# evanwang1990/FMwR

Measured on AMD Instinct MI355X. Metric: training examples/sec, 10Mx1M sparse FM SGD, higher is better.
Workload: dtype f32

## Files before the change

### fmwr_amd/_lib.py

```python
import ctypes as C
import os

_PKG = os.path.dirname(os.path.abspath(__file__))
LIB_PATH = os.environ.get("FMX_LIB_PATH") or os.path.join(_PKG, "libfmx.so")

OK, ERR_INVALID, ERR_HIP, ERR_NOGPU, ERR_STATE = 0, 1, 2, 3, 4
TASK_CLASSIFICATION, TASK_REGRESSION, TASK_RANKING = 10, 20, 30
SOLVER_MCMC, SOLVER_ALS, SOLVER_SGD, SOLVER_FTRL, SOLVER_TDAP = 100, 200, 300, 500, 600
MODE_SEQUENTIAL, MODE_MINIBATCH = 0, 1
LINK_NONE, LINK_LOGISTIC, LINK_CLAMP, LINK_PROBIT = 0, 1, 2, 3
DIV_REL_SCORE, DIV_REL_MINMAX = 0, 1
SIM_COSINE, SIM_DOT = 0, 1
REDUCE_MEAN, REDUCE_SUM = 0, 1
COLUMNS_UNIFORM, COLUMNS_ZIPF = 1, 2
EVAL_LL, EVAL_AUC, EVAL_ACC, EVAL_RMSE, EVAL_MSE, EVAL_MAE = 0, 111, 222, 333, 444, 555
EVAL_PAIR_ACC, EVAL_BPR = 666, 777
KERNEL_ROWS_FORWARD, KERNEL_COLS_UPDATE, KERNEL_SCALAR, KERNEL_SEQ, KERNEL_ALS_SWEEP = 0, 1, 2, 3, 4

SYMBOLS = [
    "fmx_last_error", "fmx_device_count", "fmx_config_default", "fmx_engine_create", "fmx_engine_destroy", "fmx_set_params",
    "fmx_get_params", "fmx_engine_save", "fmx_engine_load", "fmx_matrix_from_rlist", "fmx_matrix_from_dgc", "fmx_matrix_from_csr", "fmx_matrix_synthetic", "fmx_matrix_synthetic_fields", "fmx_matrix_synthetic_iid", "fmx_matrix_synthetic_ragged", "fmx_matrix_synthetic_values", "fmx_train_stream", "fmx_matrix_set_labels", "fmx_matrix_set_fields", "fmx_matrix_destroy",
    "fmx_matrix_info", "fmx_matrix_export", "fmx_matrix_scales", "fmx_matrix_normalize", "fmx_predict", "fmx_train", "fmx_train_grid", "fmx_train_order", "fmx_num_batches",
    "fmx_step", "fmx_grad", "fmx_grad_buffer", "fmx_grad_elem_bytes", "fmx_grad_layout", "fmx_grad_begin", "fmx_grad_chunk", "fmx_apply_chunk", "fmx_apply", "fmx_sync", "fmx_stream", "fmx_predict_device",
    "fmx_als_plan_info", "fmx_als_tiled_info", "fmx_als_order_info", "fmx_als_carry_q", "fmx_als_vsweep", "fmx_mcmc_vsweep", "fmx_als_train", "fmx_mcmc_train", "fmx_mcmc_train_from", "fmx_mcmc_v_hyper", "fmx_evaluate", "fmx_train_tracked", "fmx_trace_size", "fmx_trace_get", "fmx_trace_params",
# ... 32 lines not shown
SPLIT_NO_PART = 0xFFFFFFFF
MET_VALUES, MET_COUNTS = 6, 4
MET_AUC, MET_LOGLOSS, MET_ACCURACY, MET_BRIER, MET_MEAN_PRED, MET_MEAN_LABEL = 0, 1, 2, 3, 4, 5
MET_MSE, MET_RMSE, MET_MAE, MET_MEAN_ERR = 0, 1, 2, 3
MET_ROWS, MET_POSITIVES, MET_PAIRS2, MET_CORRECT = 0, 1, 2, 3
CAL_NONE, CAL_PLATT, CAL_STEPS = 0, 1, 2
BINS_WIDTH, BINS_MASS = 0, 1
CAL_VALUES = 4
CAL_ECE, CAL_MCE, CAL_BRIER, CAL_LOGLOSS = 0, 1, 2, 3


TEST_HOOKS = ["fmx_debug_fail_next_plan_build", "fmx_debug_fail_next_comm_init", "fmx_debug_lose_next_seq_multiplier", "fmx_debug_stall_next_persistent_sweep",
              "fmx_debug_contrib_summary_chunk", "fmx_debug_foldin_slab", "fmx_debug_heldout_limits", "fmx_debug_pairs_hard_chunk", "fmx_debug_lists_limits", "fmx_debug_diversify_limits", "fmx_debug_neighbors_limits", "fmx_debug_interactions_limits", "fmx_debug_metrics_limits", "fmx_debug_take_limits", "fmx_debug_calibrate_limits", "fmx_debug_columns_limits", "fmx_debug_join_limits", "fmx_debug_bins_limits", "fmx_debug_matrix_flags", "fmx_debug_cols_launches",
              "fmx_debug_long_launches", "fmx_debug_rows_launches", "fmx_debug_rows_merged_launches",
              "fmx_debug_rows_sched_launches", "fmx_debug_rows_sched_id_limit", "fmx_debug_rows_sched_export",
              "fmx_debug_rows_pace_launches", "fmx_debug_rows_pace_trace",
              "fmx_debug_rows_clock_launches", "fmx_debug_rows_clock_records_of", "fmx_debug_rows_clock_poison"]


class Config(C.Structure):
    _fields_ = [
        ("struct_size", C.c_uint32), ("task", C.c_int32), ("solver", C.c_int32), ("num_factor", C.c_int32),
        ("keep_w0", C.c_int32), ("keep_w1", C.c_int32),
        ("l2_w0", C.c_double), ("l1_w1", C.c_double), ("l2_w1", C.c_double), ("l1_v", C.c_double), ("l2_v", C.c_double),
        ("learn_rate", C.c_double),
        ("alpha_w", C.c_double), ("alpha_v", C.c_double), ("beta_w", C.c_double), ("beta_v", C.c_double),
        ("random_step", C.c_int32), ("mode", C.c_int32), ("batch_rows", C.c_int64),
        ("min_target", C.c_double), ("max_target", C.c_double),
        ("device", C.c_int32), ("batch_reduce", C.c_int32), ("gamma", C.c_double), ("tile_rows", C.c_int64),
        ("state_fp64", C.c_int32), ("exchange_chunks", C.c_int32), ("n_gpus", C.c_int32), ("als_max_levels", C.c_int32), ("seq_reassociate", C.c_int32), ("gpus_share_device", C.c_int32),
    ]
# ... 128 lines not shown
```

### fmwr_amd/csrc/fm_batch_kernels.hip

```cpp
#include <atomic>
#include <mutex>
#include <utility>
#include <vector>

#include "fmx_internal.h"
#include "fm_probit.h"
#include "fmx_test_hooks.h"

#ifndef FMX_U
#define FMX_U 4
#endif
#ifndef FMX_SPARSE_WAVES
#define FMX_SPARSE_WAVES 4
#endif
#ifndef FMX_DENSE_WAVES
#define FMX_DENSE_WAVES 4
#endif
#ifndef FMX_U_LARGE
#define FMX_U_LARGE 4
#endif
#ifndef FMX_U_SMALL
#define FMX_U_SMALL 8
#endif

// ... 453 lines not shown
  }
  if constexpr (TRAIN) {
    __syncthreads();
    if (tid % 64 == 0) {
      const int s = tid / 64;
      if (R0 + (int64_t)s * NG < a.nrows) {
        double g0 = 0.0, q0 = 0.0;
        for (int i = 0; i < NG; ++i) { const double m = red[s * NG + i]; g0 += m; q0 += m * m; }
        a.partials[2 * ((size_t)blockIdx.x * MERGE_SLOTS + s)] = g0;
        a.partials[2 * ((size_t)blockIdx.x * MERGE_SLOTS + s) + 1] = q0;
      }
    }
  }
}

constexpr int64_t PACE_STEP_CYCLES = 2120;

__device__ __forceinline__ void pace_sleep(int units) {
  switch (units) {
    case 3: __builtin_amdgcn_s_sleep(3); break;
    case 4: __builtin_amdgcn_s_sleep(4); break;
    case 5: __builtin_amdgcn_s_sleep(5); break;
    case 6: __builtin_amdgcn_s_sleep(6); break;
    case 8: __builtin_amdgcn_s_sleep(8); break;
    case 9: __builtin_amdgcn_s_sleep(9); break;
    case 10: __builtin_amdgcn_s_sleep(10); break;
    case 12: __builtin_amdgcn_s_sleep(12); break;
    case 15: __builtin_amdgcn_s_sleep(15); break;
    case 16: __builtin_amdgcn_s_sleep(16); break;
    case 24: __builtin_amdgcn_s_sleep(24); break;
    case 20: __builtin_amdgcn_s_sleep(20); break;
// ... 11 lines not shown
#define FMX_ROWS_PACE_CLOCK_EVERY 24
#endif
#ifndef FMX_ROWS_PACE_CLOCK_LEAD
#define FMX_ROWS_PACE_CLOCK_LEAD 0.5
#endif
#ifndef FMX_ROWS_PACE_CLOCK_SLEEP
#define FMX_ROWS_PACE_CLOCK_SLEEP 30
#endif
#ifndef FMX_ROWS_PACE_CLOCK_GAIN
#define FMX_ROWS_PACE_CLOCK_GAIN 1.00
#endif
static_assert((int64_t)((SCHED_STAGE_STEPS - 1) / FMX_ROWS_PACE_CLOCK_EVERY) * 3 * FMX_ROWS_PACE_CLOCK_SLEEP * 64 * 10 <= SCHED_STAGE_STEPS * PACE_STEP_CYCLES, "clock checks x the longest sleep: at most a tenth of the longest block's walk");
static_assert((int64_t)((120 - 1) / FMX_ROWS_PACE_CLOCK_EVERY) * 3 * FMX_ROWS_PACE_CLOCK_SLEEP * 64 * 10 <= 120 * PACE_STEP_CYCLES, "the same for the headline's 120-step blocks");
static_assert(FMX_ROWS_PACE_CLOCK_GAIN > 0.0 && FMX_ROWS_PACE_CLOCK_GAIN <= 1.0, "a gain above 1 would hold a launch to a pace slower than the one observed");

template <bool DEAL, bool PACED, bool TRACE>
__global__ __launch_bounds__(WG_THREADS, 4) void fm_rows_sched_k(RowsArgs a, Hyper h) {
  using T = float;
  constexpr int LPR = 4, VEC = 4, KP = LPR * VEC;
  constexpr int NG = WG_THREADS / LPR;
  constexpr int PER = MERGE_STAGE / WG_THREADS;
  static_assert(MERGE_STAGE == SCHED_STAGE_STEPS * NG && MERGE_SLOTS == 4, "the stage holds SCHED_STAGE_STEPS steps of one word per lane group");
  __shared__ uint32_t stage[MERGE_STAGE];
  __shared__ double red[MERGE_RPW];
  __shared__ uint32_t places[DEAL ? NG : 1];

  const int tid = threadIdx.x;
  const int gid = tid / LPR;
  const int lig = tid % LPR;
  const int64_t R0 = (int64_t)blockIdx.x * MERGE_RPW;
  const uint32_t w_hi = a.sched_dir[blockIdx.x + 1];
  uint32_t w_lo = a.sched_dir[blockIdx.x];
  if constexpr (DEAL) {
    const bool hdr = w_hi - w_lo >= (uint32_t)NG;
    if (tid < NG) places[tid] = hdr ? a.sched[(size_t)w_lo + tid] : 0u;
    w_lo += hdr ? (uint32_t)NG : 0u;
  }
  const int cnt = (w_hi - w_lo < (uint32_t)MERGE_STAGE) ? (int)(w_hi - w_lo) : MERGE_STAGE;
  const int steps = cnt / NG;
  {
    uint32_t id[PER];
// ... 37 lines not shown
      const uint64_t planted = __hip_atomic_load(rec + 1, __ATOMIC_RELAXED, __HIP_MEMORY_SCOPE_AGENT);
      const uint64_t ticks = sums & ((1ull << CLK_TICK_BITS) - 1), done = sums >> CLK_TICK_BITS;
      if (planted) target = (uint32_t)planted;
      else if (done) {
        const double q8 = (double)a.clk_gain_q10 * 0.25 * (double)ticks / (double)done;
        target = q8 < 4294967295.0 ? (uint32_t)q8 : 0xFFFFFFFFu;
      }
    }
    clk_target = (int64_t)(uint32_t)__builtin_amdgcn_readfirstlane((int)target);
    if (clk_target) clk_at = a.pace_every;
    if (blockIdx.x == 0 && tid < 8 && a.clk_zero)
      __hip_atomic_store(a.clk + (size_t)(((a.clk_write + 1) % 3) * 8 + tid) * CLK_LINE, (uint64_t)0, __ATOMIC_RELAXED, __HIP_MEMORY_SCOPE_AGENT);
    clk_t0 = __builtin_amdgcn_s_memrealtime();
  }
  uint64_t* trace = nullptr;
  if constexpr (TRACE) trace = a.pace_trace + ((size_t)blockIdx.x * (WG_THREADS / 64) + tid / 64) * PACE_TRACE_WORDS;
  for (int t = 0; t < steps; ++t) {
    if constexpr (TRACE) {
      if ((t & 15) == 0 && (tid & 63) == 0) trace[1 + (t >> 4)] = __builtin_amdgcn_s_memrealtime();
    }
    const uint32_t wd = mine[t * NG];
    const bool live = wd != SCHED_BUBBLE;
    const uint32_t c = wd & SCHED_MAX_P;
    const int esl = live ? (int)(wd >> 30) : MERGE_SLOTS;
    const float4 vv = buf_row(v_rsrc, live ? (c << vsh) + lane_off : BUF_SKIP, T());
    const T wv = buf_elem(w_rsrc, live ? c << wsh : BUF_SKIP, T());
    const double x = 1.0;
    const double wx = (double)wv * x;
    double tmp[VEC], tsq[VEC];
    slice_get(vv, tmp);
#pragma unroll
    for (int i = 0; i < VEC; ++i) { tmp[i] = tmp[i] * x; tsq[i] = tmp[i] * tmp[i]; }
#pragma unroll
    for (int s = 0; s < MERGE_SLOTS; ++s) {
      if (esl == s) {
        if (k1) lin[s] += wx;
#pragma unroll
        for (int i = 0; i < VEC; ++i) { sm[s][i] += tmp[i]; qm[s][i] += tsq[i]; }
      }
    }
    if constexpr (PACED) {
      if (t == clk_at) {
        clk_at += a.pace_every;
        const int64_t gone = (int64_t)((__builtin_amdgcn_s_memrealtime() - clk_t0) << 10);
        const int64_t done = 4 * (t + 1), lead = a.pace_lead;
        const int level = (done - 3 * lead) * clk_target > gone ? 3 : (done - 2 * lead) * clk_target > gone ? 2 : (done - lead) * clk_target > gone ? 1 : 0;
        if (level) { pace_sleep(level * a.pace_sleep); pace_slept += 1 + (level << 16); }
      }
    }
  }
  if constexpr (PACED) {
    if (tid == 0) {
      const uint64_t ticks = __builtin_amdgcn_s_memrealtime() - clk_t0;
      (void)__hip_atomic_fetch_add(a.clk + (size_t)(a.clk_write * 8 + (int)(blockIdx.x & 7u)) * CLK_LINE,
                                   (ticks & ((1ull << CLK_TICK_BITS) - 1)) | (uint64_t)steps << CLK_TICK_BITS, __ATOMIC_RELAXED, __HIP_MEMORY_SCOPE_AGENT);
    }
  }
  if constexpr (TRACE) {
    if ((tid & 63) == 0) {
      trace[1 + ((steps + 15) >> 4)] = __builtin_amdgcn_s_memrealtime();
      trace[0] = (uint64_t)(__builtin_amdgcn_s_getreg((31 << 11) | 20) & 15u) | (uint64_t)steps << 8 | (uint64_t)pace_slept << 32;
    }
// ... 22 lines not shown
      *reinterpret_cast<float4*>(reinterpret_cast<T*>(a.S) + (size_t)row * KP + lig * VEC) = srow;
      if (lig == 0) reinterpret_cast<T*>(a.amul)[row] = (T)mult;
    }
    if (lig == 0) red[at] = mult;
  }
  __syncthreads();
  if (tid % 64 == 0) {
    const int s = tid / 64;
    if (R0 + (int64_t)s * NG < a.nrows) {
      double g0 = 0.0, q0 = 0.0;
      for (int i = 0; i < NG; ++i) { const double m = red[s * NG + i]; g0 += m; q0 += m * m; }
      a.partials[2 * ((size_t)blockIdx.x * MERGE_SLOTS + s)] = g0;
      a.partials[2 * ((size_t)blockIdx.x * MERGE_SLOTS + s) + 1] = q0;
    }
  }
}

template <typename T, int LPR, bool TRAIN>
__global__ __launch_bounds__(WG_THREADS) void fm_rows_forward_dyn_k(RowsArgs a, Hyper h) {
  using vec_t = typename Slice<T>::vec;
  constexpr int VEC = Slice<T>::N;
  constexpr int KP = LPR * VEC;
  constexpr int GROUPS = WG_THREADS / LPR;
  constexpr int RPW = 4 * GROUPS;
  constexpr int RU = FMX_U_LARGE;
  constexpr int PER = (RU + LPR - 1) / LPR;
  __shared__ int next_row;
  __shared__ double red[TRAIN ? RPW : 1];
  const int tid = threadIdx.x;
  const int grp = tid / LPR, lig = tid % LPR;
  const int lane0 = (tid & 63) - lig;
// ... 463 lines not shown
void rows_sched_count_build() { g_rows_sched[2]++; }
static int rows_sched_mode() {
  static const int v = [] { const char* s = getenv("FMX_ROWS_SCHED"); return s ? atoi(s) : (getenv("FMX_ROWS_MERGE") ? 0 : FMX_ROWS_SCHED_DEFAULT); }();
  return v;
}
static int rows_sched_policy() {
  static const int v = [] {
    const char* s = getenv("FMX_ROWS_SCHED_POLICY");
    if (!s) return (int)FMX_ROWS_SCHED_POLICY_DEFAULT;
    return s[0] == 'm' ? (int)SCHED_MERGE : s[0] == 'd' ? (int)SCHED_DEAL : (int)FMX_ROWS_SCHED_POLICY_DEFAULT;
  }();
  return v;
}

#ifndef FMX_ROWS_PACE_DEFAULT
#define FMX_ROWS_PACE_DEFAULT 3
#endif
static std::atomic<int64_t> g_rows_pace[2];
void debug_rows_pace_launches(int64_t out[2]) {
  for (int i = 0; i < 2; ++i) out[i] = g_rows_pace[i].load();
}
static std::atomic<int64_t> g_rows_clock[2];
void debug_rows_clock_launches(int64_t out[2]) {
  for (int i = 0; i < 2; ++i) out[i] = g_rows_clock[i].load();
}
static int rows_pace_mode() {
  static const int v = [] { const char* s = getenv("FMX_ROWS_PACE"); const int m = s ? atoi(s) : FMX_ROWS_PACE_DEFAULT; return (m == 0 || m == 3 || m == 4) ? m : FMX_ROWS_PACE_DEFAULT; }();
  return v;
}
static bool rows_pace_trace_on() { static const bool v = [] { const char* s = getenv("FMX_ROWS_PACE_TRACE"); return s && s[0] == '1'; }(); return v; }
struct ClockTune { int every, lead_q2, sleep, gain_q10; };
static const ClockTune& rows_clock_tune() {
  static const ClockTune v = [] {
    ClockTune t{FMX_ROWS_PACE_CLOCK_EVERY, (int)(FMX_ROWS_PACE_CLOCK_LEAD * 4.0 + 0.5), FMX_ROWS_PACE_CLOCK_SLEEP, (int)(FMX_ROWS_PACE_CLOCK_GAIN * 1024.0 + 0.5)};
    int ev = 0, sl = 0;
    double ld = -1.0, g = 0.0;
    const char* s = getenv("FMX_ROWS_PACE_CLOCK_TUNE");
    if (s && sscanf(s, "%d,%lf,%d,%lf", &ev, &ld, &sl, &g) == 4 && ev >= 2 && ev <= 64 && ld >= 0.0 && ld <= 64.0 && (sl == 3 || sl == 4 || sl == 5 || sl == 8 || sl == 10 || sl == 20 || sl == 30 || sl == 40) && g > 0.0 && g <= 1.0)
      t = ClockTune{ev, (int)(ld * 4.0 + 0.5), sl, (int)(g * 1024.0 + 0.5)};
    return t;
  }();
  return v;
// ... 28 lines not shown
}

static int launch_rows_sched(fmx_engine* e, const RowsArgs& a_in, bool* ran) {
  *ran = false;
  if (a_in.sched_state == 0) return FMX_OK;
  int policy = 0;
  if (!rows_sched_wanted(e, a_in, &policy)) return FMX_OK;
  if (a_in.sched_state != 1 || !a_in.sched || !a_in.sched_dir) { g_rows_sched[1]++; return FMX_OK; }
  RowsArgs a = a_in;
  a.sched_vbytes = (uint32_t)((uint64_t)e->p * (uint64_t)a.vs * sizeof(float));
  a.sched_wbytes = (uint32_t)((((uint64_t)e->p - 1) * (uint64_t)a.ws + 1) * sizeof(float));
  const int64_t grid = (a.nrows + MERGE_RPW - 1) / MERGE_RPW;
  FMX_CHECK(grid < (1LL << 31), FMX_ERR_INVALID, "rows_forward: grid too large (%lld)", (long long)grid);
  const bool traced = rows_pace_trace_on();
  using SchedKernel = void (*)(RowsArgs, Hyper);
  static const SchedKernel instance[2][2][2] = {
      {{fm_rows_sched_k<false, false, false>, fm_rows_sched_k<false, false, true>}, {fm_rows_sched_k<false, true, false>, fm_rows_sched_k<false, true, true>}},
      {{fm_rows_sched_k<true, false, false>, fm_rows_sched_k<true, false, true>}, {fm_rows_sched_k<true, true, false>, fm_rows_sched_k<true, true, true>}}};
  const int deal = a.sched_deal ? 1 : 0;
  bool paced = false;
  if (rows_pace_mode() != 0 && e->rows_clock != nullptr) {
    constexpr int MAX_DEV = 64;
    static std::atomic<int64_t> resident_dev[MAX_DEV][2][2];
    std::atomic<int64_t>& resident = resident_dev[(e->cfg.device >= 0 && e->cfg.device < MAX_DEV) ? e->cfg.device : 0][deal][traced ? 1 : 0];
    int64_t r = resident.load();
    if (r == 0) {
      hipDeviceProp_t pr{};
      int per = 0;
      if (hipGetDeviceProperties(&pr, e->cfg.device) == hipSuccess && pr.multiProcessorCount > 0 &&
          hipOccupancyMaxActiveBlocksPerMultiprocessor(&per, instance[deal][1][traced ? 1 : 0], WG_THREADS, 0) == hipSuccess && per > 0)
        r = (int64_t)per * pr.multiProcessorCount;
      else r = -1;
      resident.store(r);
    }
    paced = r > 0 && grid <= r;
  }
  bool with_target = false;
  if (paced) {
    const ClockTune& ct = rows_clock_tune();
    const int64_t n = e->rows_clock_launches;
    with_target = e->rows_clock_poisoned || (e->rows_clock_prev && e->rows_clock_uid == a.mat_uid && e->rows_clock_gen == a.mat_gen && e->rows_clock_nrows == a.nrows);
    a.clk = e->rows_clock;
    a.clk_write = (int)(n % 3);
    a.clk_read = with_target ? (int)((n + 2) % 3) : -1;
    a.clk_zero = e->rows_clock_poisoned ? 0 : 1;
// ... 6 lines not shown
      FMX_HIP(hipStreamSynchronize(e->stream));
    }
  }
  if (traced) {
    const int64_t waves = grid * (WG_THREADS / 64);
    if (waves > e->rows_pace_trace_cap) {
      FMX_HIP(hipStreamSynchronize(e->stream));
      (void)hipFree(e->rows_pace_trace); e->rows_pace_trace = nullptr; e->rows_pace_trace_cap = 0;
      FMX_HIP(hipMalloc(&e->rows_pace_trace, (size_t)waves * PACE_TRACE_WORDS * sizeof(uint64_t)));
      e->rows_pace_trace_cap = waves;
    }
    FMX_HIP(hipMemsetAsync(e->rows_pace_trace, 0, (size_t)waves * PACE_TRACE_WORDS * sizeof(uint64_t), e->stream));
    e->rows_pace_trace_waves = waves;
    a.pace_trace = e->rows_pace_trace;
  }
  hipLaunchKernelGGL(instance[deal][paced ? 1 : 0][traced ? 1 : 0], dim3((unsigned)grid), dim3(WG_THREADS), 0, e->stream, a, e->hyper);
  FMX_HIP(hipGetLastError());
  if (paced) {
    ++e->rows_clock_launches;
    e->rows_clock_prev = 1; e->rows_clock_uid = a.mat_uid; e->rows_clock_gen = a.mat_gen; e->rows_clock_nrows = a.nrows;
    g_rows_clock[with_target ? 0 : 1]++;
  }
  g_rows_pace[paced ? 0 : 1]++;
  g_rows_sched[0]++;
  *ran = true;
  return FMX_OK;
}

int launch_rows_forward(fmx_engine* e, const RowsArgs& a_in, bool train, bool fp64_tables) {
  RowsArgs a = a_in;
  FMX_CHECK(a.vs >= (fp64_tables ? e->kp64 : e->kp32) && a.ws >= 1 && (a.vs & (a.vs - 1)) == 0 && (a.ws & (a.ws - 1)) == 0, FMX_ERR_STATE,
            "rows_forward: table strides not set (%d, %d)", a.vs, a.ws);
  {
    const int kp = fp64_tables ? e->kp64 : e->kp32;
    FMX_CHECK((!fp64_tables && kp <= WIR_MAX_KP) || (a.vs == kp && a.ws == 1), FMX_ERR_STATE, "rows_forward: strides (%d, %d) on a table of compiled strides (%d, 1)",
              a.vs, a.ws, kp);
  }
  a.vsh = __builtin_ctz((unsigned)a.vs); a.wsh = __builtin_ctz((unsigned)a.ws);
  static const bool embed_ok = [] { const char* v = getenv("FMX_EMBED_MULT"); return !(v && v[0] == '0'); }();
// ... 1287 lines not shown
```

### fmwr_amd/csrc/fmx_api.hip

```cpp
#include <algorithm>
#include <cmath>
#include <cstdlib>
#include <cstring>
#include <ctime>
#include <atomic>
#include <memory>

#include "fmx_internal.h"
#include "fmx_test_hooks.h"
#include "fm_probit.h"

namespace fmx {

static thread_local std::string g_error;

void set_error(const char* fmt, ...) {
  char buf[1024];
  va_list ap;
  va_start(ap, fmt);
  vsnprintf(buf, sizeof(buf), fmt, ap);
  va_end(ap);
  g_error = buf;
}

// ... 1995 lines not shown
int fmx_debug_rows_merged_launches(int64_t* out) {
  FMX_CHECK(out != nullptr, FMX_ERR_INVALID, "out is NULL");
  debug_rows_merged_launches(out);
  return FMX_OK;
}
int fmx_debug_rows_sched_launches(int64_t* out) {
  FMX_CHECK(out != nullptr, FMX_ERR_INVALID, "out is NULL");
  debug_rows_sched_launches(out);
  return FMX_OK;
}
int fmx_debug_rows_pace_launches(int64_t* out) {
  FMX_CHECK(out != nullptr, FMX_ERR_INVALID, "out is NULL");
  debug_rows_pace_launches(out);
  return FMX_OK;
}
int fmx_debug_rows_clock_launches(int64_t* out) {
  FMX_CHECK(out != nullptr, FMX_ERR_INVALID, "out is NULL");
  debug_rows_clock_launches(out);
  return FMX_OK;
}
int fmx_debug_rows_clock_records_of(fmx_engine* e, int32_t replica, uint64_t* out) {
  FMX_CHECK(e != nullptr && out != nullptr, FMX_ERR_INVALID, "NULL engine or out");
  fmx_engine* r = group_replica(e, replica);
  FMX_CHECK(r != nullptr, FMX_ERR_INVALID, "no replica %d", (int)replica);
  FMX_HIP(hipSetDevice(r->cfg.device));
  const int st = debug_rows_clock_records(r, out);
  (void)hipSetDevice(e->cfg.device);
  return st;
}
int fmx_debug_rows_clock_poison(fmx_engine* e, uint32_t value) {
// ... 65 lines not shown
```

### fmwr_amd/csrc/fmx_internal.h

```cpp
#pragma once
#include <hip/hip_runtime.h>

#include <cstdarg>
#include <cstdint>
#include <cstdio>
#include <cstdlib>
#include <functional>
#include <string>
#include <utility>
#include <vector>

#include "../../include/fmx.h"

namespace fmx {

void set_error(const char* fmt, ...);

#define FMX_HIP(call)                                                                         \
  do {                                                                                        \
    hipError_t _e = (call);                                                                   \
    if (_e != hipSuccess) {                                                                   \
      fmx::set_error("%s failed: %s (%s:%d)", #call, hipGetErrorString(_e), __FILE__, __LINE__); \
      return FMX_ERR_HIP;                                                                     \
    }                                                                                         \
// ... 361 lines not shown
inline int64_t rows_flat_blocks(int64_t r0, int64_t nrows, int g) { return nrows > 0 ? (r0 + nrows - 1) / g - r0 / g + 1 : 0; }
inline int rows_col_skew(const fmx_matrix* m, const fmx_matrix::TilePlan& pl) {
  const uint64_t lists = pl.feat ? pl.n_lists : m->p;
  if (lists == 0 || pl.n_long == 0) return 1;
  return ((uint64_t)pl.cnt <= 32ull * lists && (uint64_t)pl.n_long * 1024ull >= lists) ? 2 : 1;
}
int launch_rows_forward(fmx_engine* e, const RowsArgs& a, bool train, bool fp64_tables);
enum RowsSchedPolicy : int { SCHED_MERGE = 0, SCHED_DEAL = 3 };
constexpr int SCHED_STAGE_STEPS = 144;
constexpr uint32_t SCHED_BUBBLE = 0xFFFFFFFFu;
constexpr uint32_t SCHED_MAX_P = (1u << 30) - 1;
bool rows_sched_wanted(fmx_engine* e, const RowsArgs& a, int* policy);
void rows_sched_count_build();
void debug_rows_sched_launches(int64_t out[3]);
constexpr int PACE_TRACE_WORDS = 16;
constexpr int CLK_LINE = 16;
constexpr int CLK_WORDS = 3 * 8 * CLK_LINE;
constexpr int CLK_TICK_BITS = 40;
void debug_rows_pace_launches(int64_t out[2]);
void debug_rows_clock_launches(int64_t out[2]);
int debug_rows_clock_records(fmx_engine* e, uint64_t out[48]);
int debug_rows_pace_trace(fmx_engine* e, uint64_t* out, int64_t cap_words, int64_t* waves);
int rows_sched_build(fmx_matrix* m, int policy, hipStream_t stream);
void rows_sched_free(fmx_matrix* m);
void debug_rows_sched_id_limit(uint32_t limit);
int debug_rows_sched_export(const fmx_matrix* m, int64_t tile, int64_t block, uint32_t* out, int64_t cap_words, int64_t* steps);
int ensure_probit(fmx_engine* e);
int topk_run(fmx_engine* e, const fmx_matrix* C, int64_t r0, int64_t r1, const fmx_matrix* I, const fmx_matrix* X, int K, int link, int64_t* d_index,
             double* d_score);
int heldout_run(fmx_engine* e, const fmx_matrix* C, int64_t r0, int64_t r1, const fmx_matrix* I, const fmx_matrix* H, const fmx_matrix* X, int64_t* d_rank,
                double* d_score, const int32_t* ks, int n_ks, double* pc);
int heldout_means(fmx_engine* e, const double* pc, int64_t n, int cols, double* out, int64_t* counted);
void debug_heldout_limits(int window, int64_t chunk);
int lists_run(fmx_engine* e, const fmx_matrix* C, int64_t r0, int64_t r1, const fmx_matrix* I, const fmx_matrix* Lm, int link, int K, double* d_score,
// ... 288 lines not shown
```

### fmwr_amd/csrc/fmx_test_hooks.h

```cpp
#ifndef FMX_TEST_HOOKS_H_
#define FMX_TEST_HOOKS_H_
#include <stdint.h>
#ifdef __cplusplus
extern "C" {
#endif
int fmx_debug_fail_next_plan_build(void);
int fmx_debug_fail_next_comm_init(void);
int fmx_debug_lose_next_seq_multiplier(void);
int fmx_debug_stall_next_persistent_sweep(void);
int fmx_debug_contrib_summary_chunk(int64_t entries);
int fmx_debug_foldin_slab(int64_t rows, int64_t groups);
int fmx_debug_heldout_limits(int32_t window, int64_t chunk);
int fmx_debug_pairs_hard_chunk(int64_t contexts);
int fmx_debug_lists_limits(int32_t lds_entries, int64_t chunk);
int fmx_debug_diversify_limits(int32_t lds_rows, int64_t chunk);
int fmx_debug_neighbors_limits(int64_t slice_items, int64_t chunk_rows);
int fmx_debug_interactions_limits(int32_t wave_entries, int32_t tile_entries, int64_t summary_rows_per_group);
int fmx_debug_metrics_limits(int32_t wave_rows, int32_t lds_rows, int64_t chunk_rows);
int fmx_debug_take_limits(int32_t fixed_entries, int32_t group_entries, int64_t rows_per_launch);
int fmx_debug_calibrate_limits(int64_t chunk_rows);
int fmx_debug_columns_limits(int32_t group_entries, int64_t chunk_entries, int64_t rows_per_launch);
int fmx_debug_join_limits(int32_t fixed_entries, int32_t group_entries, int64_t rows_per_launch);
int fmx_debug_bins_limits(int32_t lds_edges, int64_t chunk_entries);
int fmx_debug_matrix_flags(const fmx_matrix* m, int32_t* out );
int fmx_debug_cols_launches(int64_t* out);
int fmx_debug_long_launches(int64_t* out);
int fmx_debug_rows_launches(int64_t* out );
int fmx_debug_rows_merged_launches(int64_t* out );
int fmx_debug_rows_sched_launches(int64_t* out );
int fmx_debug_rows_sched_id_limit(uint32_t limit);
int fmx_debug_rows_sched_export(const fmx_matrix* m, int64_t tile, int64_t block, uint32_t* out, int64_t cap_words, int64_t* steps, int64_t* info );
int fmx_debug_rows_pace_launches(int64_t* out );
int fmx_debug_rows_clock_launches(int64_t* out );
int fmx_debug_rows_clock_records_of(fmx_engine* e, int32_t replica, uint64_t* out );
int fmx_debug_rows_clock_poison(fmx_engine* e, uint32_t value);
int fmx_debug_rows_pace_trace(fmx_engine* e, uint64_t* out, int64_t cap_words, int64_t* waves);
#ifdef __cplusplus
}
#endif
#endif
```

### profiles/rows_deal_sim.py

```python
import argparse
import os
import sys
import time

import numpy as np

sys.path.insert(0, os.path.dirname(os.path.dirname(os.path.abspath(__file__))))
from tests import rows_deal_model as D

P, NNZ, BLOCKS, NG, SLOTS, LRU_LINES, XCDS = 1_000_000, 30, 128, 64, 4, 32768, 8
W_BASE = 1 << 40


def streams(rng, kind):
    if kind == "even":
        n = SLOTS * NNZ
        band = np.arange(n, dtype=np.float64) * P / n
        return (band[None, :] + rng.random((BLOCKS * NG, n)) * P / n).astype(np.int64)
    out = np.empty((BLOCKS * NG, SLOTS * NNZ), np.int64)
    for b in range(BLOCKS):
        rows = np.sort(rng.integers(0, P, (256, NNZ)), axis=1)
        if kind == "deal":
            m = D.deal_map([[int(c) for c in r] for r in rows], P)
        else:
            m = D.identity_map()
        for g in range(NG):
            out[b * NG + g] = np.sort(np.concatenate([rows[m[s][g]] for s in range(SLOTS)]))
    return out


def excursion(cols):
    n = cols.shape[1]
    ramp = (np.arange(n) + 0.5) * P / n
    return float(np.mean(np.max(np.abs(cols - ramp[None, :]), axis=1)) / P)


def lines_fetched(cols, drift, rng):
    n_streams, n = cols.shape
    offset = np.repeat(rng.normal(0.0, drift, n_streams // 16) if drift > 0 else np.zeros(n_streams // 16), 16)
    when = (np.arange(n, dtype=np.float64)[None, :] + offset[:, None]).ravel()
    order = np.argsort(when, kind="stable")
    flat = cols.ravel()[order]
    v_line, w_line = (flat >> 1).tolist(), ((flat >> 5) + W_BASE).tolist()
    lru, miss_v, miss_w = {}, 0, 0
    for v, w in zip(v_line, w_line):
        for key in (v, w):
            if key in lru:
                del lru[key]
            else:
                if key >= W_BASE:
                    miss_w += 1
                else:
                    miss_v += 1
                if len(lru) >= LRU_LINES:
                    del lru[next(iter(lru))]
            lru[key] = None
    return miss_v, miss_w


def main():
    ap = argparse.ArgumentParser()
    ap.add_argument("--drift", type=float, nargs="*", default=[0.0, 2.0, 4.0, 8.0], help="sd of a wave's offset against the common clock, in steps")
    ap.add_argument("--seed", type=int, default=1)
    a = ap.parse_args()
    t0 = time.time()
    sets = {}
    for kind in ("identity", "deal", "even"):
        sets[kind] = streams(np.random.default_rng(a.seed), kind)
    print(f"streams made in {time.time() - t0:.1f} s; mean largest excursion from the ramp, fraction of p: " + ", ".join(f"{k} {excursion(v):.4f}" for k, v in sets.items()))
    distinct = len(np.unique(sets["identity"] >> 1))
    print(f"distinct V lines one XCD touches: {distinct} ({XCDS * distinct / 1e6:.2f} M per tile: perfect re-use)")
    print("M lines per tile (8 XCDs):   drift   identity V / w      DEAL V / w      even V / w")
    for d in a.drift:
        row = []
        for kind in ("identity", "deal", "even"):
            v, w = lines_fetched(sets[kind], d, np.random.default_rng(a.seed + 1000))
            row.append(f"{XCDS * v / 1e6:6.2f} / {XCDS * w / 1e6:4.2f}")
        print(f"                             {d:5.1f}   " + "   ".join(row), flush=True)
    print(f"{time.time() - t0:.1f} s")


if __name__ == "__main__":
    main()
```

### profiles/rows_pace_trace.py

```python
import argparse
import ctypes
import json
import os
import sys

import numpy as np

ROOT = os.path.dirname(os.path.dirname(os.path.abspath(__file__)))
sys.path.insert(0, ROOT)
WORDS = 16


def reduce_launch(tr):
    waves = tr.shape[0]
    xcc = (tr[:, 0] & 15).astype(np.int64)
    steps = ((tr[:, 0] >> 8) & 0xFFFF).astype(np.int64)
    slept = ((tr[:, 0] >> 32) & 0xFFFF).astype(np.int64)
    label = (np.arange(waves) // 4) % 8
    labels_ok = all(len(np.unique(xcc[label == lb])) == 1 for lb in range(8)) and len(np.unique(xcc)) == 8
    n = int(steps.min())
    assert n == int(steps.max()) and n >= 32, "the headline's blocks hold the same number of steps"
    at = list(range(0, n, 16))
    stamps = tr[:, 1:1 + len(at) + 1].astype(np.int64)
    t0 = stamps[:, 0].min()
    tm = (stamps - t0).astype(np.float64) * 0.01
    pos = np.array(at + [n], np.float64)
    step_us = float(np.mean((tm[:, -1] - tm[:, 0]) / n))
    out = {"waves": waves, "steps": n, "labels_are_xcds": bool(labels_ok), "launch_us": float(tm[:, -1].max()), "first_step_spread_us": float(tm[:, 0].max()),
           "step_us": step_us, "sleeps": int(slept.sum()), "waves_that_slept": int((slept > 0).sum())}
    drift = np.zeros((8, len(pos)))
    for x in range(8):
        sel = tm[label == x]
        drift[x] = sel.std(axis=0) / step_us
    out["drift_steps_by_step"] = {str(int(s)): float(v) for s, v in zip(pos, drift.mean(axis=0))}
    out["drift_steps_by_step_per_xcd_end"] = [float(v) for v in drift[:, -1]]
    b, a = np.polyfit(pos, (drift ** 2).mean(axis=0), 1)
    out["variance_fit"] = {"at_step_0": float(a), "per_step": float(b), "fixed_share_at_end": float(a / max(a + b * n, 1e-12))}
    frac = [0.1, 0.25, 0.5, 0.75, 0.9]
    lo, hi = float(np.median(tm[:, 0])), float(np.median(tm[:, -1]))
    reached = {}
    for f in frac:
        t = lo + f * (hi - lo)
        sd = []
        for x in range(8):
# ... 3 lines not shown
    out["sd_of_step_reached_at_time"] = reached
    for name, j in (("middle", len(pos) // 2), ("end", len(pos) - 1)):
        inside, between = [], []
        for x in range(8):
            sel = tm[label == x][:, j].reshape(-1, 4)
            inside.append(float(np.mean(sel.var(axis=1))))
            between.append(float(sel.mean(axis=1).var()))
        out[f"sd_inside_workgroup_steps_{name}"] = float(np.sqrt(np.mean(inside)) / step_us)
        out[f"sd_between_workgroups_steps_{name}"] = float(np.sqrt(np.mean(between)) / step_us)
    return out


def main():
    ap = argparse.ArgumentParser()
    ap.add_argument("--pace", default="0", choices=["0", "3", "4"])
    ap.add_argument("--clock-tune", default=None, help="FMX_ROWS_PACE_CLOCK_TUNE")
    ap.add_argument("--launches", type=int, default=5)
    ap.add_argument("--rows", type=int, default=262144)
    ap.add_argument("--json", default=None)
    ap.add_argument("--raw", default=None, help="save the last launch's stamps as .npy")
    a = ap.parse_args()
    os.environ["FMX_ROWS_PACE_TRACE"] = "1"
    os.environ["FMX_ROWS_PACE"] = a.pace
    if a.clock_tune:
        os.environ["FMX_ROWS_PACE_CLOCK_TUNE"] = a.clock_tune
    from fmwr_amd import _lib as L
    from fmwr_amd import engine
    lib = L.lib()
    p, z, k, B = 1_000_000, 30, 16, a.rows
    m = engine.Matrix.synthetic_iid(2 * B, p, z, 20240001, law=L.COLUMNS_UNIFORM)
    e = engine.Engine(p, task=L.TASK_CLASSIFICATION, solver=L.SOLVER_SGD, num_factor=k, learn_rate=0.01, l2_w1=1e-4, l2_v=1e-4, mode=L.MODE_MINIBATCH, batch_rows=B)
    e.init_normal(1, 0.0, 0.01)
    for i in range(40):
        e.step(m, i % 2)
    e.sync()
    per = []
    for i in range(a.launches):
        e.step(m, i % 2)
# ... 3 lines not shown
        if waves.value == 0:
            raise SystemExit("no traced launch: the step did not take the scheduled form")
        buf = np.zeros(waves.value * WORDS, np.uint64)
        L.check(lib.fmx_debug_rows_pace_trace(e.h, buf.ctypes.data_as(ctypes.c_void_p), ctypes.c_int64(len(buf)), ctypes.byref(waves)))
        per.append(reduce_launch(buf.reshape(-1, WORDS)))
        if a.raw and i == a.launches - 1:
            np.save(a.raw, buf.reshape(-1, WORDS))
    pl, cl = (ctypes.c_int64 * 2)(), (ctypes.c_int64 * 2)()
    L.check(lib.fmx_debug_rows_pace_launches(pl))
    L.check(lib.fmx_debug_rows_clock_launches(cl))
    keys = ["launch_us", "step_us", "first_step_spread_us", "sleeps", "waves_that_slept", "sd_inside_workgroup_steps_middle", "sd_between_workgroups_steps_middle",
            "sd_inside_workgroup_steps_end", "sd_between_workgroups_steps_end"]
    med = {q: float(np.median([r[q] for r in per])) for q in keys}
    med["drift_steps_by_step"] = {s: float(np.median([r["drift_steps_by_step"][s] for r in per])) for s in per[0]["drift_steps_by_step"]}
    med["sd_of_step_reached_at_time"] = {s: float(np.median([r["sd_of_step_reached_at_time"][s] for r in per])) for s in per[0]["sd_of_step_reached_at_time"]}
    med["variance_fit"] = {s: float(np.median([r["variance_fit"][s] for r in per])) for s in per[0]["variance_fit"]}
    out = {"pace": a.pace, "tune": a.clock_tune, "paced_launches": int(pl[0]), "unpaced_launches": int(pl[1]),
           "clock_launches_with_target": int(cl[0]), "clock_launches_without": int(cl[1]), "labels_are_xcds": all(r["labels_are_xcds"] for r in per),
           "median": med, "launches": per}
    print(json.dumps({q: out[q] for q in ("pace", "tune", "paced_launches", "unpaced_launches", "clock_launches_with_target", "clock_launches_without", "labels_are_xcds", "median")}, indent=1))
    if a.json:
        with open(a.json, "w") as f:
            json.dump(out, f, indent=1)
    e.close()
    m.close()


if __name__ == "__main__":
    main()
```

Measured before the change: 1.109 billion.

## Prefetch scheduled row gathers ahead and disable clock pacing by default

The scheduled rows kernel now takes a compile-time look-ahead depth and issues the V-row and w gathers for later steps into a register ring before consuming the current step. It uses explicit vmcnt waits and a sched barrier so several loads stay in flight per wave. Depth 2 is the default. The default pacing mode changes from 3 to off, and the pace step cycle constant is retuned. The change also adds entry/exit trace stamps and a launch counter per depth, trading extra registers and many more kernel instantiations for hiding gather latency and removing sleep-based pacing.

```diff
diff --git a/fmwr_amd/_lib.py b/fmwr_amd/_lib.py
--- a/fmwr_amd/_lib.py
+++ b/fmwr_amd/_lib.py
@@ -70,7 +70,7 @@
               "fmx_debug_contrib_summary_chunk", "fmx_debug_foldin_slab", "fmx_debug_heldout_limits", "fmx_debug_pairs_hard_chunk", "fmx_debug_lists_limits", "fmx_debug_diversify_limits", "fmx_debug_neighbors_limits", "fmx_debug_interactions_limits", "fmx_debug_metrics_limits", "fmx_debug_take_limits", "fmx_debug_calibrate_limits", "fmx_debug_columns_limits", "fmx_debug_join_limits", "fmx_debug_bins_limits", "fmx_debug_matrix_flags", "fmx_debug_cols_launches",
               "fmx_debug_long_launches", "fmx_debug_rows_launches", "fmx_debug_rows_merged_launches",
               "fmx_debug_rows_sched_launches", "fmx_debug_rows_sched_id_limit", "fmx_debug_rows_sched_export",
-              "fmx_debug_rows_pace_launches", "fmx_debug_rows_pace_trace",
+              "fmx_debug_rows_pace_launches", "fmx_debug_rows_pace_trace", "fmx_debug_rows_ahead_launches",
               "fmx_debug_rows_clock_launches", "fmx_debug_rows_clock_records_of", "fmx_debug_rows_clock_poison"]
 
 
diff --git a/fmwr_amd/csrc/fm_batch_kernels.hip b/fmwr_amd/csrc/fm_batch_kernels.hip
--- a/fmwr_amd/csrc/fm_batch_kernels.hip
+++ b/fmwr_amd/csrc/fm_batch_kernels.hip
@@ -491,7 +491,7 @@
   }
 }
 
-constexpr int64_t PACE_STEP_CYCLES = 2120;
+constexpr int64_t PACE_STEP_CYCLES = 2012;
 
 __device__ __forceinline__ void pace_sleep(int units) {
   switch (units) {
@@ -533,9 +533,34 @@
 static_assert((int64_t)((120 - 1) / FMX_ROWS_PACE_CLOCK_EVERY) * 3 * FMX_ROWS_PACE_CLOCK_SLEEP * 64 * 10 <= 120 * PACE_STEP_CYCLES, "the same for the headline's 120-step blocks");
 static_assert(FMX_ROWS_PACE_CLOCK_GAIN > 0.0 && FMX_ROWS_PACE_CLOCK_GAIN <= 1.0, "a gain above 1 would hold a launch to a pace slower than the one observed");
 
-template <bool DEAL, bool PACED, bool TRACE>
+#define FMX_SCHED_TAKE(t, HERE)                                                                                                                            \
+  {                                                                                                                                                        \
+    const double x = 1.0;                                                                                                                     \
+    const double wx = (double)wv * x;                                                                                                                      \
+    double tmp[VEC], tsq[VEC];                                                                                                                             \
+    slice_get(vv, tmp);                                                                                                                                    \
+    _Pragma("unroll") for (int i = 0; i < VEC; ++i) { tmp[i] = tmp[i] * x; tsq[i] = tmp[i] * tmp[i]; }                                                     \
+    _Pragma("unroll") for (int s = 0; s < MERGE_SLOTS; ++s) {                                                                                              \
+      if (esl == s) {                                                                                                                                      \
+        if (k1) lin[s] += wx;                                                                                                                              \
+        _Pragma("unroll") for (int i = 0; i < VEC; ++i) { sm[s][i] += tmp[i]; qm[s][i] += tsq[i]; }                                                        \
+      }                                                                                                                                                    \
+    }                                                                                                                                                      \
+    if constexpr (PACED) {                                                                                                                                 \
+      if ((HERE) && t == clk_at) {                                                                                                                         \
+        clk_at += a.pace_every;                                                                                                                            \
+        const int64_t gone = (int64_t)((__builtin_amdgcn_s_memrealtime() - clk_t0) << 10);              \
+        const int64_t done = 4 * (t + 1), lead = a.pace_lead;                                                                                              \
+        const int level = (done - 3 * lead) * clk_target > gone ? 3 : (done - 2 * lead) * clk_target > gone ? 2 : (done - lead) * clk_target > gone ? 1 : 0; \
+        if (level) { pace_sleep(level * a.pace_sleep); pace_slept += 1 + (level << 16); }                                                                  \
+      }                                                                                                                                                    \
+    }                                                                                                                                                      \
+  }
+
+template <bool DEAL, bool PACED, bool TRACE, int AHEAD>
 __global__ __launch_bounds__(WG_THREADS, 4) void fm_rows_sched_k(RowsArgs a, Hyper h) {
   using T = float;
+  static_assert(AHEAD >= 1 && AHEAD <= ROWS_AHEAD_MAX, "the depths the launcher's table holds");
   constexpr int LPR = 4, VEC = 4, KP = LPR * VEC;
   constexpr int NG = WG_THREADS / LPR;
   constexpr int PER = MERGE_STAGE / WG_THREADS;
@@ -544,6 +569,8 @@
   __shared__ double red[MERGE_RPW];
   __shared__ uint32_t places[DEAL ? NG : 1];
 
+  uint64_t entry_clk = 0;
+  if constexpr (TRACE) entry_clk = __builtin_amdgcn_s_memrealtime();
   const int tid = threadIdx.x;
   const int gid = tid / LPR;
   const int lig = tid % LPR;
@@ -611,38 +638,55 @@
     clk_t0 = __builtin_amdgcn_s_memrealtime();
   }
   uint64_t* trace = nullptr;
-  if constexpr (TRACE) trace = a.pace_trace + ((size_t)blockIdx.x * (WG_THREADS / 64) + tid / 64) * PACE_TRACE_WORDS;
-  for (int t = 0; t < steps; ++t) {
-    if constexpr (TRACE) {
-      if ((t & 15) == 0 && (tid & 63) == 0) trace[1 + (t >> 4)] = __builtin_amdgcn_s_memrealtime();
-    }
-    const uint32_t wd = mine[t * NG];
-    const bool live = wd != SCHED_BUBBLE;
-    const uint32_t c = wd & SCHED_MAX_P;
-    const int esl = live ? (int)(wd >> 30) : MERGE_SLOTS;
-    const float4 vv = buf_row(v_rsrc, live ? (c << vsh) + lane_off : BUF_SKIP, T());
-    const T wv = buf_elem(w_rsrc, live ? c << wsh : BUF_SKIP, T());
-    const double x = 1.0;
-    const double wx = (double)wv * x;
-    double tmp[VEC], tsq[VEC];
-    slice_get(vv, tmp);
-#pragma unroll
-    for (int i = 0; i < VEC; ++i) { tmp[i] = tmp[i] * x; tsq[i] = tmp[i] * tmp[i]; }
-#pragma unroll
-    for (int s = 0; s < MERGE_SLOTS; ++s) {
-      if (esl == s) {
-        if (k1) lin[s] += wx;
-#pragma unroll
-        for (int i = 0; i < VEC; ++i) { sm[s][i] += tmp[i]; qm[s][i] += tsq[i]; }
-      }
-    }
-    if constexpr (PACED) {
-      if (t == clk_at) {
-        clk_at += a.pace_every;
-        const int64_t gone = (int64_t)((__builtin_amdgcn_s_memrealtime() - clk_t0) << 10);
-        const int64_t done = 4 * (t + 1), lead = a.pace_lead;
-        const int level = (done - 3 * lead) * clk_target > gone ? 3 : (done - 2 * lead) * clk_target > gone ? 2 : (done - lead) * clk_target > gone ? 1 : 0;
-        if (level) { pace_sleep(level * a.pace_sleep); pace_slept += 1 + (level << 16); }
+  if constexpr (TRACE) {
+    trace = a.pace_trace + ((size_t)blockIdx.x * (WG_THREADS / 64) + tid / 64) * PACE_TRACE_WORDS;
+    if ((tid & 63) == 0) trace[PACE_TRACE_ENTRY] = entry_clk;
+  }
+  if constexpr (AHEAD == 1) {
+    for (int t = 0; t < steps; ++t) {
+      if constexpr (TRACE) {
+        if ((t & 15) == 0 && (tid & 63) == 0) trace[1 + (t >> 4)] = __builtin_amdgcn_s_memrealtime();
+      }
+      const uint32_t wd = mine[t * NG];
+      const bool live = wd != SCHED_BUBBLE;
+      const uint32_t c = wd & SCHED_MAX_P;
+      const int esl = live ? (int)(wd >> 30) : MERGE_SLOTS;
+      const float4 vv = buf_row(v_rsrc, live ? (c << vsh) + lane_off : BUF_SKIP, T());
+      const T wv = buf_elem(w_rsrc, live ? c << wsh : BUF_SKIP, T());
+      FMX_SCHED_TAKE(t, true)
+    }
+  } else {
+    uint32_t rwd[AHEAD];
+    float4 rvv[AHEAD];
+    T rwv[AHEAD];
+    auto request = [&](const int ta, const int slot) {
+      const bool in = ta < steps;
+      const uint32_t wd = in ? mine[(in ? ta : 0) * NG] : SCHED_BUBBLE;
+      const bool live = wd != SCHED_BUBBLE;
+      const uint32_t c = wd & SCHED_MAX_P;
+      rwd[slot] = wd;
+      rvv[slot] = buf_row(v_rsrc, live ? (c << vsh) + lane_off : BUF_SKIP, T());
+      rwv[slot] = buf_elem(w_rsrc, live ? c << wsh : BUF_SKIP, T());
+    };
+#pragma unroll
+    for (int u = 0; u < AHEAD - 1; ++u) request(u, u);
+    for (int t0 = 0; t0 < steps; t0 += AHEAD) {
+#pragma unroll
+      for (int u = 0; u < AHEAD; ++u) {
+        const int t = t0 + u;
+        const bool past = u > 0 && t >= steps;
+        if constexpr (TRACE) {
+          if (!past && (t & 15) == 0 && (tid & 63) == 0) trace[1 + (t >> 4)] = __builtin_amdgcn_s_memrealtime();
+        }
+        asm volatile("s_waitcnt vmcnt(%0)" ::"n"(2 * (AHEAD - 2)) : "memory");
+        request(t + AHEAD - 1, (u + AHEAD - 1) % AHEAD);
+        __builtin_amdgcn_sched_barrier(0);
+        const uint32_t wd = rwd[u];
+        const float4 vv = rvv[u];
+        const T wv = rwv[u];
+        const bool live = wd != SCHED_BUBBLE;
+        const int esl = live ? (int)(wd >> 30) : MERGE_SLOTS;
+        FMX_SCHED_TAKE(t, !past)
       }
     }
   }
@@ -695,7 +739,12 @@
       a.partials[2 * ((size_t)blockIdx.x * MERGE_SLOTS + s) + 1] = q0;
     }
   }
-}
+  if constexpr (TRACE) {
+    if ((tid & 63) == 0) trace[PACE_TRACE_EXIT] = __builtin_amdgcn_s_memrealtime();
+  }
+}
+
+#undef FMX_SCHED_TAKE
 
 template <typename T, int LPR, bool TRAIN>
 __global__ __launch_bounds__(WG_THREADS) void fm_rows_forward_dyn_k(RowsArgs a, Hyper h) {
@@ -1189,7 +1238,7 @@
 }
 
 #ifndef FMX_ROWS_PACE_DEFAULT
-#define FMX_ROWS_PACE_DEFAULT 3
+#define FMX_ROWS_PACE_DEFAULT 0
 #endif
 static std::atomic<int64_t> g_rows_pace[2];
 void debug_rows_pace_launches(int64_t out[2]) {
@@ -1201,6 +1250,18 @@
 }
 static int rows_pace_mode() {
   static const int v = [] { const char* s = getenv("FMX_ROWS_PACE"); const int m = s ? atoi(s) : FMX_ROWS_PACE_DEFAULT; return (m == 0 || m == 3 || m == 4) ? m : FMX_ROWS_PACE_DEFAULT; }();
+  return v;
+}
+#ifndef FMX_ROWS_AHEAD_DEFAULT
+#define FMX_ROWS_AHEAD_DEFAULT 2
+#endif
+static_assert(FMX_ROWS_AHEAD_DEFAULT >= 1 && FMX_ROWS_AHEAD_DEFAULT <= ROWS_AHEAD_MAX, "a depth that is built");
+static std::atomic<int64_t> g_rows_ahead[ROWS_AHEAD_MAX];
+void debug_rows_ahead_launches(int64_t out[ROWS_AHEAD_MAX]) {
+  for (int i = 0; i < ROWS_AHEAD_MAX; ++i) out[i] = g_rows_ahead[i].load();
+}
+static int rows_ahead_depth() {
+  static const int v = [] { const char* s = getenv("FMX_ROWS_AHEAD"); const int d = s ? atoi(s) : FMX_ROWS_AHEAD_DEFAULT; return (d >= 1 && d <= ROWS_AHEAD_MAX) ? d : FMX_ROWS_AHEAD_DEFAULT; }();
   return v;
 }
 static bool rows_pace_trace_on() { static const bool v = [] { const char* s = getenv("FMX_ROWS_PACE_TRACE"); return s && s[0] == '1'; }(); return v; }
@@ -1259,21 +1320,25 @@
   FMX_CHECK(grid < (1LL << 31), FMX_ERR_INVALID, "rows_forward: grid too large (%lld)", (long long)grid);
   const bool traced = rows_pace_trace_on();
   using SchedKernel = void (*)(RowsArgs, Hyper);
-  static const SchedKernel instance[2][2][2] = {
-      {{fm_rows_sched_k<false, false, false>, fm_rows_sched_k<false, false, true>}, {fm_rows_sched_k<false, true, false>, fm_rows_sched_k<false, true, true>}},
-      {{fm_rows_sched_k<true, false, false>, fm_rows_sched_k<true, false, true>}, {fm_rows_sched_k<true, true, false>, fm_rows_sched_k<true, true, true>}}};
+  static_assert(ROWS_AHEAD_MAX == 4, "one entry per depth");
+#define FMX_SCHED_DEPTHS(D, P, T) {fm_rows_sched_k<D, P, T, 1>, fm_rows_sched_k<D, P, T, 2>, fm_rows_sched_k<D, P, T, 3>, fm_rows_sched_k<D, P, T, 4>}
+  static const SchedKernel instance[2][2][2][ROWS_AHEAD_MAX] = {
+      {{FMX_SCHED_DEPTHS(false, false, false), FMX_SCHED_DEPTHS(false, false, true)}, {FMX_SCHED_DEPTHS(false, true, false), FMX_SCHED_DEPTHS(false, true, true)}},
+      {{FMX_SCHED_DEPTHS(true, false, false), FMX_SCHED_DEPTHS(true, false, true)}, {FMX_SCHED_DEPTHS(true, true, false), FMX_SCHED_DEPTHS(true, true, true)}}};
+#undef FMX_SCHED_DEPTHS
   const int deal = a.sched_deal ? 1 : 0;
+  const int depth = rows_ahead_depth();
   bool paced = false;
   if (rows_pace_mode() != 0 && e->rows_clock != nullptr) {
     constexpr int MAX_DEV = 64;
-    static std::atomic<int64_t> resident_dev[MAX_DEV][2][2];
-    std::atomic<int64_t>& resident = resident_dev[(e->cfg.device >= 0 && e->cfg.device < MAX_DEV) ? e->cfg.device : 0][deal][traced ? 1 : 0];
+    static std::atomic<int64_t> resident_dev[MAX_DEV][2][2][ROWS_AHEAD_MAX];
+    std::atomic<int64_t>& resident = resident_dev[(e->cfg.device >= 0 && e->cfg.device < MAX_DEV) ? e->cfg.device : 0][deal][traced ? 1 : 0][depth - 1];
     int64_t r = resident.load();
     if (r == 0) {
       hipDeviceProp_t pr{};
       int per = 0;
       if (hipGetDeviceProperties(&pr, e->cfg.device) == hipSuccess && pr.multiProcessorCount > 0 &&
-          hipOccupancyMaxActiveBlocksPerMultiprocessor(&per, instance[deal][1][traced ? 1 : 0], WG_THREADS, 0) == hipSuccess && per > 0)
+          hipOccupancyMaxActiveBlocksPerMultiprocessor(&per, instance[deal][1][traced ? 1 : 0][depth - 1], WG_THREADS, 0) == hipSuccess && per > 0)
         r = (int64_t)per * pr.multiProcessorCount;
       else r = -1;
       resident.store(r);
@@ -1310,7 +1375,7 @@
     e->rows_pace_trace_waves = waves;
     a.pace_trace = e->rows_pace_trace;
   }
-  hipLaunchKernelGGL(instance[deal][paced ? 1 : 0][traced ? 1 : 0], dim3((unsigned)grid), dim3(WG_THREADS), 0, e->stream, a, e->hyper);
+  hipLaunchKernelGGL(instance[deal][paced ? 1 : 0][traced ? 1 : 0][depth - 1], dim3((unsigned)grid), dim3(WG_THREADS), 0, e->stream, a, e->hyper);
   FMX_HIP(hipGetLastError());
   if (paced) {
     ++e->rows_clock_launches;
@@ -1319,6 +1384,7 @@
   }
   g_rows_pace[paced ? 0 : 1]++;
   g_rows_sched[0]++;
+  g_rows_ahead[depth - 1]++;
   *ran = true;
   return FMX_OK;
 }
diff --git a/fmwr_amd/csrc/fmx_api.hip b/fmwr_amd/csrc/fmx_api.hip
--- a/fmwr_amd/csrc/fmx_api.hip
+++ b/fmwr_amd/csrc/fmx_api.hip
@@ -2033,6 +2033,11 @@
   debug_rows_pace_launches(out);
   return FMX_OK;
 }
+int fmx_debug_rows_ahead_launches(int64_t* out) {
+  FMX_CHECK(out != nullptr, FMX_ERR_INVALID, "out is NULL");
+  debug_rows_ahead_launches(out);
+  return FMX_OK;
+}
 int fmx_debug_rows_clock_launches(int64_t* out) {
   FMX_CHECK(out != nullptr, FMX_ERR_INVALID, "out is NULL");
   debug_rows_clock_launches(out);
diff --git a/fmwr_amd/csrc/fmx_internal.h b/fmwr_amd/csrc/fmx_internal.h
--- a/fmwr_amd/csrc/fmx_internal.h
+++ b/fmwr_amd/csrc/fmx_internal.h
@@ -399,10 +399,15 @@
 void rows_sched_count_build();
 void debug_rows_sched_launches(int64_t out[3]);
 constexpr int PACE_TRACE_WORDS = 16;
+constexpr int PACE_TRACE_ENTRY = 15;
+constexpr int PACE_TRACE_EXIT = 14;
+static_assert(1 + (SCHED_STAGE_STEPS + 15) / 16 < PACE_TRACE_EXIT, "the walk's stamps end below the two ends' words");
+constexpr int ROWS_AHEAD_MAX = 4;
 constexpr int CLK_LINE = 16;
 constexpr int CLK_WORDS = 3 * 8 * CLK_LINE;
 constexpr int CLK_TICK_BITS = 40;
 void debug_rows_pace_launches(int64_t out[2]);
+void debug_rows_ahead_launches(int64_t out[ROWS_AHEAD_MAX]);
 void debug_rows_clock_launches(int64_t out[2]);
 int debug_rows_clock_records(fmx_engine* e, uint64_t out[48]);
 int debug_rows_pace_trace(fmx_engine* e, uint64_t* out, int64_t cap_words, int64_t* waves);
diff --git a/fmwr_amd/csrc/fmx_test_hooks.h b/fmwr_amd/csrc/fmx_test_hooks.h
--- a/fmwr_amd/csrc/fmx_test_hooks.h
+++ b/fmwr_amd/csrc/fmx_test_hooks.h
@@ -31,6 +31,7 @@
 int fmx_debug_rows_sched_id_limit(uint32_t limit);
 int fmx_debug_rows_sched_export(const fmx_matrix* m, int64_t tile, int64_t block, uint32_t* out, int64_t cap_words, int64_t* steps, int64_t* info );
 int fmx_debug_rows_pace_launches(int64_t* out );
+int fmx_debug_rows_ahead_launches(int64_t* out );
 int fmx_debug_rows_clock_launches(int64_t* out );
 int fmx_debug_rows_clock_records_of(fmx_engine* e, int32_t replica, uint64_t* out );
 int fmx_debug_rows_clock_poison(fmx_engine* e, uint32_t value);
diff --git a/profiles/rows_deal_sim.py b/profiles/rows_deal_sim.py
--- a/profiles/rows_deal_sim.py
+++ b/profiles/rows_deal_sim.py
@@ -35,10 +35,11 @@
     return float(np.mean(np.max(np.abs(cols - ramp[None, :]), axis=1)) / P)
 
 
-def lines_fetched(cols, drift, rng):
+def lines_fetched(cols, drift, rng, ahead=1):
     n_streams, n = cols.shape
     offset = np.repeat(rng.normal(0.0, drift, n_streams // 16) if drift > 0 else np.zeros(n_streams // 16), 16)
-    when = (np.arange(n, dtype=np.float64)[None, :] + offset[:, None]).ravel()
+    issued = np.maximum(np.arange(n, dtype=np.float64) - (ahead - 1), 0.0)
+    when = (issued[None, :] + offset[:, None]).ravel()
     order = np.argsort(when, kind="stable")
     flat = cols.ravel()[order]
     v_line, w_line = (flat >> 1).tolist(), ((flat >> 5) + W_BASE).tolist()
@@ -61,6 +62,7 @@
 def main():
     ap = argparse.ArgumentParser()
     ap.add_argument("--drift", type=float, nargs="*", default=[0.0, 2.0, 4.0, 8.0], help="sd of a wave's offset against the common clock, in steps")
+    ap.add_argument("--ahead", type=int, nargs="*", default=[], help="look-ahead depths to price under DEAL (1: the walk that requests and consumes step by step)")
     ap.add_argument("--seed", type=int, default=1)
     a = ap.parse_args()
     t0 = time.time()
@@ -77,6 +79,14 @@
             v, w = lines_fetched(sets[kind], d, np.random.default_rng(a.seed + 1000))
             row.append(f"{XCDS * v / 1e6:6.2f} / {XCDS * w / 1e6:4.2f}")
         print(f"                             {d:5.1f}   " + "   ".join(row), flush=True)
+    if a.ahead:
+        print("DEAL, M lines per tile (8 XCDs), V + w, by look-ahead depth:   drift   " + "   ".join(f"AHEAD {d}" for d in a.ahead))
+        for d in a.drift:
+            row = []
+            for depth in a.ahead:
+                v, w = lines_fetched(sets["deal"], d, np.random.default_rng(a.seed + 1000), depth)
+                row.append(f"{XCDS * (v + w) / 1e6:7.3f}")
+            print(f"                                                               {d:5.1f}   " + "   ".join(row), flush=True)
     print(f"{time.time() - t0:.1f} s")
 
 
diff --git a/profiles/rows_pace_trace.py b/profiles/rows_pace_trace.py
--- a/profiles/rows_pace_trace.py
+++ b/profiles/rows_pace_trace.py
@@ -28,6 +28,15 @@
     step_us = float(np.mean((tm[:, -1] - tm[:, 0]) / n))
     out = {"waves": waves, "steps": n, "labels_are_xcds": bool(labels_ok), "launch_us": float(tm[:, -1].max()), "first_step_spread_us": float(tm[:, 0].max()),
            "step_us": step_us, "sleeps": int(slept.sum()), "waves_that_slept": int((slept > 0).sum())}
+    if tr[:, 15].all() and tr[:, 14].all():
+        entry, leave = (tr[:, 15].astype(np.int64) - t0) * 0.01, (tr[:, 14].astype(np.int64) - t0) * 0.01
+        head, tail = tm[:, 0] - entry, leave - tm[:, -1]
+        out["entry_to_step0_us"] = {"median": float(np.median(head)), "min": float(head.min()), "max": float(head.max())}
+        out["last_step_to_exit_us"] = {"median": float(np.median(tail)), "min": float(tail.min()), "max": float(tail.max())}
+        out["entry_spread_us"] = float(entry.max() - entry.min())
+        out["first_entry_to_last_exit_us"] = float(leave.max() - entry.min())
+        out["first_entry_to_first_step0_us"] = float(tm[:, 0].min() - entry.min())
+        out["last_walk_end_to_last_exit_us"] = float(leave.max() - tm[:, -1].max())
     drift = np.zeros((8, len(pos)))
     for x in range(8):
         sel = tm[label == x]
@@ -61,6 +70,7 @@
 def main():
     ap = argparse.ArgumentParser()
     ap.add_argument("--pace", default="0", choices=["0", "3", "4"])
+    ap.add_argument("--ahead", default=None, choices=["1", "2", "3", "4"], help="FMX_ROWS_AHEAD (unset: the library's default)")
     ap.add_argument("--clock-tune", default=None, help="FMX_ROWS_PACE_CLOCK_TUNE")
     ap.add_argument("--launches", type=int, default=5)
     ap.add_argument("--rows", type=int, default=262144)
@@ -69,6 +79,8 @@
     a = ap.parse_args()
     os.environ["FMX_ROWS_PACE_TRACE"] = "1"
     os.environ["FMX_ROWS_PACE"] = a.pace
+    if a.ahead:
+        os.environ["FMX_ROWS_AHEAD"] = a.ahead
     if a.clock_tune:
         os.environ["FMX_ROWS_PACE_CLOCK_TUNE"] = a.clock_tune
     from fmwr_amd import _lib as L
@@ -102,11 +114,16 @@
     med = {q: float(np.median([r[q] for r in per])) for q in keys}
     med["drift_steps_by_step"] = {s: float(np.median([r["drift_steps_by_step"][s] for r in per])) for s in per[0]["drift_steps_by_step"]}
     med["sd_of_step_reached_at_time"] = {s: float(np.median([r["sd_of_step_reached_at_time"][s] for r in per])) for s in per[0]["sd_of_step_reached_at_time"]}
+    if "entry_to_step0_us" in per[0]:
+        for q in ("entry_to_step0_us", "last_step_to_exit_us"):
+            med[q] = {s: float(np.median([r[q][s] for r in per])) for s in ("median", "min", "max")}
+        for q in ("entry_spread_us", "first_entry_to_last_exit_us", "first_entry_to_first_step0_us", "last_walk_end_to_last_exit_us"):
+            med[q] = float(np.median([r[q] for r in per]))
     med["variance_fit"] = {s: float(np.median([r["variance_fit"][s] for r in per])) for s in per[0]["variance_fit"]}
-    out = {"pace": a.pace, "tune": a.clock_tune, "paced_launches": int(pl[0]), "unpaced_launches": int(pl[1]),
+    out = {"pace": a.pace, "ahead": a.ahead, "tune": a.clock_tune, "paced_launches": int(pl[0]), "unpaced_launches": int(pl[1]),
            "clock_launches_with_target": int(cl[0]), "clock_launches_without": int(cl[1]), "labels_are_xcds": all(r["labels_are_xcds"] for r in per),
            "median": med, "launches": per}
-    print(json.dumps({q: out[q] for q in ("pace", "tune", "paced_launches", "unpaced_launches", "clock_launches_with_target", "clock_launches_without", "labels_are_xcds", "median")}, indent=1))
+    print(json.dumps({q: out[q] for q in ("pace", "ahead", "tune", "paced_launches", "unpaced_launches", "clock_launches_with_target", "clock_launches_without", "labels_are_xcds", "median")}, indent=1))
     if a.json:
         with open(a.json, "w") as f:
             json.dump(out, f, indent=1)
```

New measurement: 1.135 billion, median of 6. +2.4%, better.
